# alexkreimer/libviso

Hardware: AMD Instinct MI355X
Metric: stereo_frames_per_sec_1241x376_matcher (higher is better)
Workload: dtype u16; 1 GPU; configs[1]: synthetic 1241x376 stereo pairs, 2000 features/image, SAD matcher only (pack + 3 match_desc/frame + sort)

## Files before the change

### libviso_amd/csrc/common.h

```cpp
#pragma once
#include <hip/hip_runtime.h>
#include <stdint.h>
#include <stddef.h>
#include <atomic>

#include "../../include/viso_hip.h"

#define VISO_ROW 128
#define VISO_ROW8 128
#define VISO_ROW8_SLACK(S) (((1 << (S)) - 1) * VISO_ROW8)
#define VISO_R8_C128 0
#define VISO_R8_ROWS 3
#define VISO_R8_DEFAULT 3
#define VISO_R8_EVERY 16
#define VISO_PACK_SUMS 1
#define VISO_PACK_ROWS8 2
#define VISO_BIAS 32768
#define VISO_WAVE 64
#define VISO_QCAP 256
#define VISO_QPB 32
#define VISO_MATCH_THREADS 256
#define VISO_KPCAP 768
#define VISO_NB 256
#define VISO_SORT_MAX 16384

void viso_set_error(const char* fmt, ...);

#define HIP_TRY(expr)                                                              \
    do {                                                                           \
        hipError_t _e = (expr);                                                    \
        if (_e != hipSuccess) {                                                    \
            viso_set_error("%s:%d: %s -> %s", __FILE__, __LINE__, #expr,           \
                           hipGetErrorString(_e));                                 \
            return VISO_ERR_HIP;                                                   \
        }                                                                          \
    } while (0)

#define VISO_TRY(expr)                                                             \
    do {                                                                           \
        const int _r = (expr);                                                     \
        if (_r < 0) return _r;                                                     \
    } while (0)

struct MatchParamsDev {
    int epi, second, K, _pad;
    float radius, _padf;
    double F[9];
    double sampson_thresh, ratio;
};

struct ImageView {
    const float2* kp;
    const float* frows;
    const int* n;
    float2* skp;
    int* sidx;
    int* rank;
    int* bstart;
    float* xinfo;
    uint8_t* qord;
    uint16_t* rows;
    uint2* sums;
    uint8_t* rows8;
    int* bad;
};

struct MatchProblem {
    ImageView q, t;
    int2* res;
    int* sorted;
    int* pos;
    int* m_cnt;
    unsigned long long* scored;
    int2* ovf;
    int* ovf_cnt;
    int* tile_flag;
    int pidx;
    int cap;
};

struct SolverParamsDev {
    double base, f, cu, cv, inlier_threshold, thresh;
    int ransac_iter, _pad;
};

enum ScratchSlot {
    SLOT_GEN0 = 0, SLOT_GEN1, SLOT_GEN2,
    SLOT_HARRIS_TMP_RESP,
    SLOT_HYP_WORDS,
    SLOT_HYP_TR,
    SLOT_GEN6,
    SLOT_HARRIS_STRIPS,
    SLOT_RANSAC_QUEUE,
    SLOT_RANSAC_ROT,
    SLOT_UNUSED10, SLOT_UNUSED11, SLOT_UNUSED12, SLOT_UNUSED13,
    SLOT_PLAIN_IN, SLOT_PLAIN_OUT,
    SLOT_CIRCLE_TAB,
    SLOT_SUBPIX_IMG, SLOT_SUBPIX_KP, SLOT_SUBPIX_LIST, SLOT_SUBPIX_UV,
// ... 351 lines not shown
```

### libviso_amd/csrc/match.hip

```cpp
#include "common.h"
#include <stdlib.h>
#include "match_dev.h"

#include <math.h>

#ifndef VISO_IMG_THREADS
#define VISO_IMG_THREADS 512
#endif
#ifndef VISO_KP_REGS
#define VISO_KP_REGS 4
#endif

#ifdef VISO_DEBUG_VARIANTS
__device__ unsigned long long viso_dbg_sortkp_clk[8];
extern "C" int viso_debug_sortkp_clocks(unsigned long long* out8) {
    (void)hipDeviceSynchronize();
    return hipMemcpyFromSymbol(out8, HIP_SYMBOL(viso_dbg_sortkp_clk), sizeof(unsigned long long) * 8, 0, hipMemcpyDeviceToHost) == hipSuccess ? VISO_OK : VISO_ERR_HIP;
}
#define SK_CLK(I) do { if (blockIdx.x == 0 && threadIdx.x == 0) viso_dbg_sortkp_clk[I] = wall_clock64(); } while (0)
#else
#define SK_CLK(I) do {} while (0)
#endif
struct KpImport2 { KpImport k[2]; };
__global__ __launch_bounds__(VISO_IMG_THREADS) void sort_kp_kernel(const ImageView* imgs, int n_img, int n64_alloc,
// ... 747 lines not shown
            const int blo = bucket_of<VISO_NB>(xa - r - slack, x0, scale);
            const int bhi = bucket_of<VISO_NB>(xb + r + slack, x0, scale);
            win.lo = P.t.bstart[blo];
            win.W = P.t.bstart[bhi + 1] - win.lo;
        }
    }
    win.cap = min(win.W, VISO_KPCAP);
    for (int w = threadIdx.x; w < win.cap; w += VISO_MATCH_THREADS) {
        s_kp[w] = P.t.skp[win.lo + w];
        s_idx[w] = P.t.sidx[win.lo + w];
    }
    float2 kp0 = make_float2(0.f, 0.f);
    const bool has0 = n2 > 0;
    if (has0) kp0 = P.t.skp[P.t.rank[0]];
    __syncthreads();
    unsigned long long scored = 0;
    for (int j = q0 + wave; j < q1; j += VISO_MATCH_WAVES) {
        QueryResult r;
        const bool done = match_query<GENERAL, false, EPI>(P, mp, j, win, kp0, has0, s_queue[wave], lane, a.dlen, scored, r);
        if (lane == 0) {
            if (done) {
                bool accept = r.idx >= 0;
                if (accept && mp.second) accept = r.bd1 < r.bd2 * mp.ratio;
                P.res[P.q.sidx[j]] = make_int2(accept ? r.idx : -1, r.dist);
            } else {
                P.ovf[atomicAdd(P.ovf_cnt, 1)] = make_int2(prob, j);
            }
        }
    }
    if (lane == 0 && scored) atomicAdd(P.scored, scored);
}

template <bool GENERAL, int EPI>
__global__ __attribute__((amdgpu_waves_per_eu(GENERAL ? 4 : 8, 8))) __launch_bounds__(VISO_MATCH_THREADS) void match_kernel(MatchArgs a) {
    __shared__ __attribute__((aligned(16))) uint2 s_queue[VISO_MATCH_WAVES][VISO_QCAP];
    __shared__ float2 s_kp[VISO_KPCAP];
    __shared__ int s_idx[VISO_KPCAP];
    __shared__ float s_xr[2];
    if constexpr (GENERAL) {
        if (*a.bad == 0) return;
        for (int vb = blockIdx.x; vb < a.vblocks; vb += gridDim.x) {
            __syncthreads();
            match_tile_slot<GENERAL, EPI>(a, vb, s_queue, s_kp, s_idx, s_xr);
        }
    } else {
        match_tile_slot<GENERAL, EPI>(a, blockIdx.x, s_queue, s_kp, s_idx, s_xr);
    }
}

#define VISO_OVF_GRID 4096
#define VISO_OVF_STAGE 768

template <bool GENERAL>
__global__ __launch_bounds__(VISO_WAVE) void match_overflow_kernel(MatchArgs a) {
    __shared__ __attribute__((aligned(16))) uint2 s_queue[VISO_QCAP];
    __shared__ __attribute__((aligned(16))) uint4 s_stage[VISO_OVF_STAGE];
    if (GENERAL && *a.bad == 0) return;
    const int n_ovf = *a.ovf_cnt;
    const int lane = threadIdx.x;
    for (int k = (int)blockIdx.x; k < n_ovf; k += (int)gridDim.x) {
        const int2 e = a.ovf_q[k];
        const MatchProblem P = a.probs[e.x];
        if (((*P.q.bad | *P.t.bad) != 0) != GENERAL) continue;
        const int j = e.y;
        const int n2 = *P.t.n;
        const MatchParamsDev& mp = a.mp[P.pidx];
        float2 kp0 = make_float2(0.f, 0.f);
        const bool has0 = n2 > 0;
        if (has0) kp0 = P.t.skp[P.t.rank[0]];
        unsigned long long scored = 0;
        Window win;
        win.gkp = P.t.skp; win.gidx = P.t.sidx; win.skp = nullptr; win.sidx = nullptr;
        win.lo = 0; win.W = 0; win.cap = 0;
        {
            const float qx = P.q.skp[j].x, r = mp.radius;
            if (n2 > 0 && r >= 0.f) {
                if (qx == qx) {
                    const float slack = (2.f * fabsf(qx) + fabsf(r)) * 1e-6f + 1e-6f;
                    const float x0 = P.t.xinfo[0], scale = P.t.xinfo[1];
                    win.lo = P.t.bstart[bucket_of<VISO_NB>(qx - r - slack, x0, scale)];
                    win.W = P.t.bstart[bucket_of<VISO_NB>(qx + r + slack, x0, scale) + 1] - win.lo;
                }
            }
        }
        QueryResult r;
        match_query<GENERAL, true, -1>(P, mp, j, win, kp0, has0, s_queue, lane, a.dlen, scored, r, s_stage, VISO_OVF_STAGE);
        if (lane == 0) {
            bool accept = r.idx >= 0;
            if (accept && mp.second) accept = r.bd1 < r.bd2 * mp.ratio;
            P.res[P.q.sidx[j]] = make_int2(accept ? r.idx : -1, r.dist);
            if (scored) atomicAdd(P.scored, scored);
        }
        __builtin_amdgcn_wave_barrier();
    }
}

const char* matcher_kernel_name(int variant) {
    return variant == 2 ? "match_batch_kernel<0>" : variant == 3 ? "match_union_kernel" : variant == 5 ? "match_prune_kernel" : variant == 6 ? "match_union8_kernel" : "match_strip_kernel";
}

int launch_match(hipStream_t s, const MatchProblem* probs_dev, int n_probs, int cap_max,
                 int dlen, const MatchParamsDev mp[2], int* bad,
                 hipEvent_t e0, hipEvent_t e1, int layout, int variant,
                 const int2* ovf_q, const int* ovf_cnt, int r8s, int general_possible, int kinds) {
    if (n_probs <= 0 || cap_max <= 0) return VISO_OK;
    variant = matcher_effective(variant, dlen);
    MatchArgs a;
    a.probs = probs_dev;
    a.n_probs = n_probs;
    a.bpp = (cap_max + VISO_QPB - 1) / VISO_QPB;
    a.dlen = dlen;
    a.gs = 1; a.gf = 0; a.gc = 1;
    a.bad = bad;
    a.ovf_q = ovf_q; a.ovf_cnt = ovf_cnt;
    a.mp[0] = mp[0];
    a.mp[1] = mp[1];
    const int groups = (n_probs + 7) / 8;
    const long long blocks = (long long)groups * 8 * a.bpp;
    if (blocks > 0x7fffffffLL) { viso_set_error("matcher grid too large"); return VISO_ERR_UNSUPPORTED; }
    a.vblocks = (int)blocks;
    if (e0) HIP_TRY(hipEventRecord(e0, s));
    {
        const int r = launch_match_batch(s, probs_dev, n_probs, cap_max, mp, bad, layout, e1, variant, r8s, kinds);
        if (r < 0) return r;
    }
    const unsigned gblocks = (unsigned)(blocks < 512 ? blocks : 512);
    if (general_possible && (kinds & VISO_KIND_ALL) == VISO_KIND_ALL) {
        hipLaunchKernelGGL((match_kernel<true, -1>), dim3(gblocks), dim3(VISO_MATCH_THREADS), 0, s, a);
        HIP_TRY(hipGetLastError());
    } else if (general_possible && (kinds & VISO_KIND_TEMPORAL)) {
        hipLaunchKernelGGL((match_kernel<true, 0>), dim3(gblocks), dim3(VISO_MATCH_THREADS), 0, s, a);
        HIP_TRY(hipGetLastError());
    } else if (general_possible && (kinds & VISO_KIND_STEREO)) {
        hipLaunchKernelGGL((match_kernel<true, 1>), dim3(gblocks), dim3(VISO_MATCH_THREADS), 0, s, a);
        HIP_TRY(hipGetLastError());
    }
    hipLaunchKernelGGL(match_overflow_kernel<false>, dim3(VISO_OVF_GRID), dim3(VISO_WAVE), 0, s, a);
    HIP_TRY(hipGetLastError());
    if (general_possible) {
        hipLaunchKernelGGL(match_overflow_kernel<true>, dim3(VISO_OVF_GRID), dim3(VISO_WAVE), 0, s, a);
        HIP_TRY(hipGetLastError());
    }
    return VISO_OK;
}


#define VISO_SORT_THREADS 512
#define VISO_SORT_NB 2048
#define VISO_SORT_FINE 1024
#define VISO_SORT_BMAX 128
#define VISO_SORT_FAST_MAX 8192

__device__ __forceinline__ void sort_tri_row(const TriItem& T, const SolverParamsDev& sp, int r, int i1, int i2) {
    const float2 a = T.kp1[i1], b = T.kp2[i2];
    const double uL = a.x, vL = a.y, uR = b.x, vR = b.y;
    T.x[0 * T.ld + r] = uL; T.x[1 * T.ld + r] = vL; T.x[2 * T.ld + r] = uR; T.x[3 * T.ld + r] = vR;
    if (T.X) {
        const double d = uL - uR;
        T.X[0 * T.ld + r] = sp.base * (uL - sp.cu) / d;
        T.X[1 * T.ld + r] = sp.base * (vL - sp.cv) / d;
        T.X[2 * T.ld + r] = sp.f * sp.base / d;
    }
}

#ifdef VISO_DEBUG_VARIANTS
__device__ unsigned long long viso_dbg_sortm_clk[12];
extern "C" int viso_debug_sortm_clocks(unsigned long long* out12) {
    (void)hipDeviceSynchronize();
    return hipMemcpyFromSymbol(out12, HIP_SYMBOL(viso_dbg_sortm_clk), sizeof(unsigned long long) * 12, 0, hipMemcpyDeviceToHost) == hipSuccess ? VISO_OK : VISO_ERR_HIP;
}
#define SM_CLK(I) do { if (blockIdx.x == 1 && threadIdx.x == 0) viso_dbg_sortm_clk[I] = wall_clock64(); } while (0)
#else
#define SM_CLK(I) do {} while (0)
#endif
__global__ __launch_bounds__(VISO_SORT_THREADS) void sort_matches_kernel(const MatchProblem* probs,
                                                                         int n_probs, int npad_alloc, int fast, int flagged_empty,
                                                                         const TriItem* tri, SolverParamsDev tri_sp) {
    extern __shared__ __attribute__((aligned(16))) unsigned char smem[];
    unsigned long long* keys = reinterpret_cast<unsigned long long*>(smem);
    __shared__ int s_cnt;
    __shared__ int s_start[VISO_SORT_NB + 1];
    __shared__ uint32_t s_red[2][VISO_SORT_THREADS / 64];
    __shared__ unsigned long long s_sum[VISO_SORT_THREADS / 64];
    __shared__ int s_maxb;
    const int prob = blockIdx.x;
    if (prob >= n_probs) return;
    SM_CLK(0);
    const MatchProblem P = probs[prob];
    const bool do_tri = tri != nullptr && prob == 0;
    TriItem T{};
    if (do_tri) T = *tri;
    if (flagged_empty && (*P.q.bad | *P.t.bad) != 0) { if (threadIdx.x == 0) *P.m_cnt = 0; return; }
    const int n1 = *P.q.n;
    const int lane = threadIdx.x & 63, wv = threadIdx.x >> 6;
    if (threadIdx.x == 0) s_cnt = 0;
// ... 109 lines not shown
                const int2 rr = P.res[i1];
                P.sorted[3 * r + 0] = i1;
                P.sorted[3 * r + 1] = rr.x;
                P.sorted[3 * r + 2] = (int)(uint32_t)(k >> 32);
                P.pos[i1] = r;
                if (do_tri) sort_tri_row(T, tri_sp, r, i1, rr.x);
            }
            SM_CLK(7);
            return;
        }
#undef SORT_BUCKET
    }
    int npad = 64;
    while (npad < mv) npad <<= 1;
    for (int i = mv + threadIdx.x; i < npad; i += VISO_SORT_THREADS) keys[i] = ~0ull;
    __syncthreads();
    bitonic_sort_lds<VISO_SORT_THREADS>(keys, npad);
    for (int r = threadIdx.x; r < mv; r += VISO_SORT_THREADS) {
        const unsigned long long k = keys[r];
        const int i1 = (int)(uint32_t)k;
        const int2 rr = P.res[i1];
        P.sorted[3 * r + 0] = i1;
        P.sorted[3 * r + 1] = rr.x;
        P.sorted[3 * r + 2] = (int)(uint32_t)(k >> 32);
        P.pos[i1] = r;
        if (do_tri) sort_tri_row(T, tri_sp, r, i1, rr.x);
    }
}

int launch_sort(hipStream_t s, const MatchProblem* probs_dev, int n_probs, int cap_max, int flagged_empty, const TriItem* tri, const SolverParamsDev* tri_sp) {
    if (n_probs <= 0) return VISO_OK;
    if (cap_max > VISO_SORT_MAX) {
        viso_set_error("match_desc: more than %d queries per call is not supported by this build", VISO_SORT_MAX);
        return VISO_ERR_UNSUPPORTED;
    }
    int npad = 64;
    while (npad < cap_max) npad <<= 1;
    const int fast = npad <= VISO_SORT_FAST_MAX ? 1 : 0;
    const size_t lds = (size_t)npad * sizeof(unsigned long long) * (fast ? 2 : 1) + 16;
    if (lds > 40 * 1024)
        HIP_TRY(hipFuncSetAttribute((const void*)sort_matches_kernel, hipFuncAttributeMaxDynamicSharedMemorySize, (int)lds));
    SolverParamsDev sp{};
    if (tri && tri_sp) sp = *tri_sp;
    hipLaunchKernelGGL(sort_matches_kernel, dim3(n_probs), dim3(VISO_SORT_THREADS), lds, s, probs_dev, n_probs, npad, fast, flagged_empty,
                       tri_sp ? tri : nullptr, sp);
    HIP_TRY(hipGetLastError());
    return VISO_OK;
}

void fill_match_params(MatchParamsDev* d, const viso_match_params* h) {
    d->epi = h->enforce_epipolar != 0;
    d->second = h->enforce_2nd_best != 0;
    d->K = h->max_neighbors;
    d->_pad = 0;
    d->radius = (float)h->radius;
    if (d->radius == 0.f) d->radius = 0.f;
    d->_padf = 0;
    for (int i = 0; i < 9; ++i) d->F[i] = h->F[i];
    d->sampson_thresh = h->sampson_thresh;
    d->ratio = h->ratio_2nd_best;
}
```

### libviso_amd/csrc/match_batch.hip

```cpp
#include "common.h"
#include <stdlib.h>
#include "match_dev.h"

#define MB_THREADS 256
#define MB_WAVES 4
#define MB_QPB 64
#define MB_G 4
#define MB_SEG 128
#define MB_PAD 32
#define MB_KPCAP 512


template <int EPI>
__global__ __attribute__((amdgpu_waves_per_eu(5, 8))) __launch_bounds__(MB_THREADS) void match_batch_kernel(BatchMatchArgs a) {
    __shared__ __attribute__((aligned(16))) uint32_t s_pairs[MB_WAVES][MB_G * MB_SEG + MB_PAD];
    __shared__ __attribute__((aligned(16))) uint32_t s_sads[MB_WAVES][MB_G * MB_SEG + MB_PAD];
    __shared__ __attribute__((aligned(16))) uint32_t s_qrow[MB_WAVES][MB_G][64];
    __shared__ float2 s_kp[MB_KPCAP];
    __shared__ int s_idx[MB_KPCAP];
    __shared__ float s_xr[4];
    if (EPI && a.bad[1] == 0) return;
    for (int vb = blockIdx.x; vb < a.vblocks; vb += gridDim.x) {
    if (vb != (int)blockIdx.x) __syncthreads();
    int prob, qblk;
// ... 236 lines not shown
                sb_ = __builtin_amdgcn_sad_u16(r0[SB].z, b0_.z, sb_);                                      \
                sa_ = __builtin_amdgcn_sad_u16(r0[SA].w, a0_.w, sa_);                                      \
                sb_ = __builtin_amdgcn_sad_u16(r0[SB].w, b0_.w, sb_);                                      \
                sa_ = __builtin_amdgcn_sad_u16(r1[SA].x, a1_.x, sa_);                                      \
                sb_ = __builtin_amdgcn_sad_u16(r1[SB].x, b1_.x, sb_);                                      \
                sa_ = __builtin_amdgcn_sad_u16(r1[SA].y, a1_.y, sa_);                                      \
                sb_ = __builtin_amdgcn_sad_u16(r1[SB].y, b1_.y, sb_);                                      \
                sa_ = __builtin_amdgcn_sad_u16(r1[SA].z, a1_.z, sa_);                                      \
                sb_ = __builtin_amdgcn_sad_u16(r1[SB].z, b1_.z, sb_);                                      \
                sa_ = __builtin_amdgcn_sad_u16(r1[SA].w, a1_.w, sa_);                                      \
                sb_ = __builtin_amdgcn_sad_u16(r1[SB].w, b1_.w, sb_);                                      \
                sa_ += wave_dpp<0xB1>(sa_);                                                                \
                sb_ += wave_dpp<0xB1>(sb_);                                                                \
                sa_ += wave_dpp<0x4E>(sa_);                                                                \
                sb_ += wave_dpp<0x4E>(sb_);                                                                \
                sa_ += wave_dpp<0x141>(sa_);                                                               \
                sb_ += wave_dpp<0x141>(sb_);                                                               \
                if (sub == 0) { sads[dst[SA]] = sa_; sads[dst[SB]] = sb_; }    \
            } while (0)
            int t = 0;
            for (; t + MB_NP < npass; t += MB_NP) {
#pragma unroll
                for (int p = 0; p < MB_NP; p += 2) {
                    MB_REDUCE2(p, p + 1);
                    MB_ISSUE(p, t + p + MB_NP);
                    MB_ISSUE(p + 1, t + p + 1 + MB_NP);
                }
            }
            if (npass > 0) {
#pragma unroll
                for (int p = 0; p < MB_NP; p += 2) MB_REDUCE2(p, p + 1);
            }
#undef MB_REDUCE2
#undef MB_ISSUE
        }
        __builtin_amdgcn_wave_barrier();
        const int nmax = max(max(seg_n[0], seg_n[1]), max(seg_n[2], seg_n[3]));
        if (EPI && nmax <= 16) {
            const int row = lane >> 4, i16 = lane & 15;
            const int n = row == 0 ? seg_n[0] : row == 1 ? seg_n[1] : row == 2 ? seg_n[2] : seg_n[3];
            const int st = row == 0 ? 0 : row == 1 ? c1 : row == 2 ? c2 : c3;
            const int my_orig = row == 0 ? orig[0] : row == 1 ? orig[1] : row == 2 ? orig[2] : orig[3];
            const bool valid = i16 < n;
            const uint32_t sv = valid ? sads[st + i16] : 0xffffffffu;
            const uint32_t m1 = row_min_u32(sv);
            const bool eq = valid && sv == m1;
            const unsigned long long em = __ballot(eq);
            const uint32_t emr = (uint32_t)(em >> (16 * row)) & 0xffffu;
            const int c = __popc(emr);
            const uint32_t m2 = row_min_u32(eq ? 0xffffffffu : sv);
            const uint32_t r_d2 = c > 1 ? m1 : m2;
            if (i16 == 0 && my_orig >= 0) {
                const int j = jg + row * MB_WAVES;
                if (((flags >> row) & 1) || (m1 != 0xffffffffu && c > 1)) {
                    P.ovf[atomicAdd(P.ovf_cnt, 1)] = make_int2(prob, j);
                } else {
                    bool accept = m1 != 0xffffffffu;
                    int idx = -1;
                    if (accept) {
                        const uint32_t r_w = (pairs[st + (__ffs((int)emr) - 1)] & 0x3fffffffu) >> 8;
                        if ((int)r_w < wcap) idx = s_idx[r_w]; else idx = P.t.sidx[lo + (int)r_w];
                        if (mp.second) {
                            const double bd2 = r_d2 == 0xffffffffu ? 1.7976931348623157e308 : (double)r_d2;
                            accept = (double)m1 < bd2 * mp.ratio;
                        }
                    }
                    P.res[my_orig] = make_int2(accept ? idx : -1, (int)m1);
                    scored += (unsigned long long)n;
                }
            }
        } else {
    #pragma unroll
            for (int k = 0; k < MB_G; ++k) {
                if (orig[k] < 0) continue;
                const int j = jg + k * MB_WAVES;
                if (flags & (1 << k)) {
                    if (lane == 0) P.ovf[atomicAdd(P.ovf_cnt, 1)] = make_int2(prob, j);
                    continue;
                }
                const int n = seg_n[k], st = k == 0 ? 0 : k == 1 ? c1 : k == 2 ? c2 : c3;
                uint32_t r_d1 = 0xffffffffu, r_d2 = 0xffffffffu, r_w = 0, r_tie = 0;
                for (int b = 0; b < n; b += VISO_WAVE) {
                    const bool valid = (b + lane) < n;
                    const uint32_t s = valid ? sads[st + b + lane] : 0xffffffffu;
                    const uint32_t m1 = wave_min_u32(s);
                    const bool eq = valid && s == m1;
                    const unsigned long long em = __ballot(eq);
                    const int c = __popcll(em);
                    const uint32_t m2 = wave_min_u32(eq ? 0xffffffffu : s);
                    const uint32_t wfirst = (pairs[st + b + (__ffsll((long long)em) - 1)] & 0x3fffffffu) >> 8;
                    const uint32_t o2 = c > 1 ? m1 : m2;
                    if (m1 < r_d1) { r_d2 = min(r_d1, o2); r_d1 = m1; r_w = wfirst; r_tie = c > 1; }
                    else if (m1 == r_d1) { r_d2 = r_d1; r_tie = 1; }
                    else r_d2 = min(r_d2, m1);
                }
                if (lane == 0) {
                    if (r_tie) {
                        P.ovf[atomicAdd(P.ovf_cnt, 1)] = make_int2(prob, j);
                    } else {
                        bool accept = r_d1 != 0xffffffffu;
                        int idx = -1;
                        if (accept) {
                            if ((int)r_w < wcap) idx = s_idx[r_w]; else idx = P.t.sidx[lo + (int)r_w];
                            if (mp.second) {
                                const double bd2 = r_d2 == 0xffffffffu ? 1.7976931348623157e308 : (double)r_d2;
                                accept = (double)r_d1 < bd2 * mp.ratio;
                            }
                        }
                        P.res[orig[k]] = make_int2(accept ? idx : -1, (int)r_d1);
                        scored += (unsigned long long)n;
                    }
                }
            }

        }
    }
    scored += (unsigned long long)__shfl_xor((long long)scored, 16);
    scored += (unsigned long long)__shfl_xor((long long)scored, 32);
    if (lane == 0 && scored) atomicAdd(P.scored, scored);
    }
}

int launch_match_batch(hipStream_t s, const MatchProblem* probs_dev, int n_probs, int cap_max,
                       const MatchParamsDev mp[2], int* bad, int layout, hipEvent_t e_mid, int variant, int r8s, int kinds) {
    BatchMatchArgs a;
    a.probs = probs_dev;
    a.n_probs = n_probs;
    a.bpp = (cap_max + MB_QPB - 1) / MB_QPB;
    a.gs = 1; a.gf = 0; a.gc = 1; a.vblocks = 0;
    a.bad = bad;
    a.r8s = r8s; a._pad8 = 0;
    a.mp[0] = mp[0];
    a.mp[1] = mp[1];
    const int groups = (n_probs + 7) / 8;
    long long bt = (long long)groups * 8 * a.bpp, bs = bt;
    BatchMatchArgs at = a, as = a;
    if (layout == 1) {
        const int g3 = (groups + 2) / 3;
        at.gs = 3; at.gf = 1; at.gc = 2; bt = (long long)g3 * 2 * 8 * a.bpp;
        as.gs = 3; as.gf = 0; as.gc = 1; bs = (long long)g3 * 8 * a.bpp;
    }
    if (bt > 0x7fffffffLL || bs > 0x7fffffffLL) { viso_set_error("matcher grid too large"); return VISO_ERR_UNSUPPORTED; }
    if (variant == 6 && (kinds & VISO_KIND_ALL) == VISO_KIND_ALL && bt <= VISO_FRAME_MAX_BLOCKS && !e_mid) {
        static const int off = [] { const char* e = getenv("VISO_FRAME_KERNEL"); return e && *e == '0'; }();
        if (!off) {
            const int r = launch_match_frame(s, at, as, bt, cap_max);
            if (r < 0) return r;
            if (kinds & VISO_KIND_NO_WIDE) return VISO_OK;
            as.vblocks = (int)bs;
            hipLaunchKernelGGL((match_batch_kernel<1>), dim3((unsigned)(bs < 1024 ? bs : 1024)), dim3(MB_THREADS), 0, s, as);
// ... 53 lines not shown
```

### libviso_amd/csrc/match_prune.hip

```cpp
#include "common.h"
#include "match_dev.h"

#define MP_THREADS 256
#define MP_WAVES 4
#define MP_QPB 64
#define MP_G 8
#ifndef MP_QSTRIDE
#define MP_QSTRIDE 64
#endif
#ifndef MP_WPE
#define MP_WPE 4
#endif
#ifndef MP_NP
#define MP_NP 2
#endif
#define MP_UCAP 448
#define MP_CCAP 480
#define MP_CPAD (8 * MP_NP + 16)
#define MP_LCAP 576
#define MP_KPCAP 512
#define MP_NBY 64

struct MpTrack { uint32_t m1, m2; };
__device__ __forceinline__ void mp_update(MpTrack& t, uint32_t key) {
// ... 353 lines not shown
        __builtin_amdgcn_wave_barrier();
        MpTrack tr;
        tr.m1 = 0xffffffffu; tr.m2 = 0xffffffffu;
        {
            const int npass = (ccnt + 7) >> 3;
            u32x4 r0[MP_NP], r1[MP_NP];
            uint32_t ent[MP_NP];
#define MP_ISSUE(SLOT, T)                                                                                  \
            do {                                                                                           \
                ent[SLOT] = cells[(T) * 8 + g8];                                                           \
                const grow_t row_ = (grow_t)(wrows + ((ent[SLOT] & 0x00ffffffu) | (uint32_t)(sub << 4)));  \
                r0[SLOT] = row_[0];                                                                        \
                r1[SLOT] = row_[8];                                                                        \
            } while (0)
#define MP_REDUCE(SLOT, T)                                                                                 \
            do {                                                                                           \
                const uint32_t k_ = ent[SLOT] >> 29;                                                       \
                const uint32_t s_sad = MP_SADROW(k_, r0[SLOT], r1[SLOT]);                                  \
                const int c_ = (T) * 8 + g8;                                                               \
                const bool mine_ = k_ == (uint32_t)sub && c_ < ccnt;                                       \
                mp_update(tr, mine_ ? ((s_sad << 9) | (uint32_t)c_) : 0xffffffffu);                        \
            } while (0)
            if (npass > 0) {
#pragma unroll
                for (int p = 0; p < MP_NP; ++p) MP_ISSUE(p, p);
            }
            int t = 0;
            for (; t + MP_NP < npass; t += MP_NP) {
#pragma unroll
                for (int p = 0; p < MP_NP; ++p) {
                    MP_REDUCE(p, t + p);
                    __builtin_amdgcn_sched_barrier(0);
                    MP_ISSUE(p, t + p + MP_NP);
                    __builtin_amdgcn_sched_barrier(0);
                }
            }
            if (npass > 0) {
#pragma unroll
                for (int p = 0; p < MP_NP; ++p) MP_REDUCE(p, t + p);
            }
#undef MP_REDUCE
#undef MP_ISSUE
        }
#pragma unroll
        for (int m = 8; m < VISO_WAVE; m <<= 1) {
            MpTrack o;
            o.m1 = (uint32_t)__shfl_xor((int)tr.m1, m);
            o.m2 = (uint32_t)__shfl_xor((int)tr.m2, m);
            mp_merge(tr, o);
        }
        if (lane < MP_G && my_orig >= 0) {
            const bool none = tr.m1 == 0xffffffffu;
            const uint32_t d1 = tr.m1 >> 9;
            const bool tie = !none && tr.m2 != 0xffffffffu && (tr.m2 >> 9) == d1;
            if (list_ovf || my_cnt > K || tie) {
                P.ovf[atomicAdd(P.ovf_cnt, 1)] = make_int2(prob, my_j);
            } else {
                bool accept = !none;
                int idx = -1;
                if (accept) {
                    const int w = (int)((cells[tr.m1 & 511u] >> 8) & 0xffffu);
                    idx = P.t.sidx[lo + w];
                    if (mp.second) {
                        const double bd2 = tr.m2 == 0xffffffffu ? 1.7976931348623157e308 : (double)(tr.m2 >> 9);
                        accept = (double)d1 < bd2 * mp.ratio;
                    }
                }
                P.res[my_orig] = make_int2(accept ? idx : -1, none ? -1 : (int)d1);
                scored += (unsigned long long)my_cnt;
            }
        }
        __builtin_amdgcn_wave_barrier();
    }
#undef MP_SADROW
#pragma unroll
    for (int m = 1; m < MP_G; m <<= 1) scored += (unsigned long long)__shfl_xor((long long)scored, m);
    if (lane == 0 && scored) atomicAdd(P.scored, scored);
}

int launch_match_prune_temporal(hipStream_t s, const BatchMatchArgs& a, long long blocks) {
    hipLaunchKernelGGL(match_prune_kernel, dim3((unsigned)blocks), dim3(MP_THREADS), 0, s, a);
    hipError_t e = hipGetLastError();
    if (e != hipSuccess) { viso_set_error("match_prune_kernel launch: %s", hipGetErrorString(e)); return VISO_ERR_HIP; }
    return VISO_OK;
}
```

### libviso_amd/csrc/match_stereo.hip

```cpp
#include "common.h"
#include "match_dev.h"

#define ST_THREADS 256
#define ST_WAVES 4
#define ST_QPW 64
#define ST_WCAP 384
#define ST_NBY 64
#define ST_SLOTS 8
#define ST_PCAP (ST_QPW * ST_SLOTS)
#ifndef ST_NP
#define ST_NP 2
#endif
#define ST_PAD (8 * ST_NP)
#define ST_BAND_MAX 6.0f

struct StWaveLds {
    float2 ykp[ST_WCAP];
    uint16_t ypos[ST_WCAP];
    int hist[ST_NBY + 1];
    uint16_t slot[ST_SLOTS][ST_QPW];
    uint32_t flat[ST_PCAP + ST_PAD];
};
static_assert(ST_WCAP <= 512, "window positions share a word with the SAD");

// ... 196 lines not shown
                    __builtin_amdgcn_sched_barrier(0);
                    ST_ISSUE(p, t + p + ST_NP);
                    __builtin_amdgcn_sched_barrier(0);
                }
            }
            if (npass > 0) {
#pragma unroll
                for (int p = 0; p < ST_NP; ++p) ST_REDUCE(p);
            }
#undef ST_REDUCE
#undef ST_ISSUE
        }
        __builtin_amdgcn_wave_barrier();
        ST_CLK(5);
        for (int s = 0; s < n2g; ++s) {
            const uint32_t f = L.flat[base + s];
            const uint32_t v = f >> 9;
            const uint32_t w = (f & 0x1ffu) + (uint32_t)cb;
            const bool lt = v < d1, eq = v == d1;
            d2 = (v <= d1) ? d1 : min(d2, v);
            bw = lt ? w : bw;
            tie = lt ? 0u : (eq ? 1u : tie);
            d1 = min(d1, v);
        }
        nscored += n2g;
        __builtin_amdgcn_wave_barrier();
        if (!__any(seen > skip + ST_SLOTS)) break;
        }
    }
    ST_CLK(6);
    int cnt = cnt_ub;
    {
        unsigned long long need = __ballot(live && cnt_ub > K);
        while (need) {
            const int ql = __ffsll((long long)need) - 1;
            need &= need - 1;
            const float qx = readlane_f32(qv.x, ql);
            const float qy = readlane_f32(qv.y, ql);
            const uint32_t th = (uint32_t)__builtin_amdgcn_readlane((int)thr, ql);
            int c = 0;
            for (int base = 0; base < W; base += VISO_WAVE) {
                const int w = base + lane;
                bool in = false;
                if (w < W) in = __float_as_uint(l1_kp(qx, qy, P.t.skp[lo + w])) < th;
                c += __popcll(__ballot(in));
            }
            if (lane == ql) cnt = c;
        }
    }
    ST_CLK(7);
    unsigned long long scored = 0;
    if (live) {
        const bool none = d1 == 0xffffffffu;
        if (cnt > K || (!none && tie)) {
            P.ovf[atomicAdd(P.ovf_cnt, 1)] = make_int2(prob, j);
        } else {
            bool accept = !none;
            int idx = -1;
            if (accept) {
                idx = P.t.sidx[lo + (int)bw];
                if (mp.second) {
                    const double bd2 = d2 == 0xffffffffu ? 1.7976931348623157e308 : (double)d2;
                    accept = (double)d1 < bd2 * mp.ratio;
                }
            }
            P.res[orig] = make_int2(accept ? idx : -1, (int)d1);
            scored = (unsigned long long)nscored;
        }
    }
    scored = viso_wave_sum63(scored);
    if (lane == 63 && scored) atomicAdd(P.scored, scored);
}

#ifndef ST_NO_LAUNCHER
int launch_match_stereo(hipStream_t s, const BatchMatchArgs& a64, int cap_max) {
    BatchMatchArgs a = a64;
    const int tiles = (cap_max + ST_QPW - 1) / ST_QPW;
    a.bpp = (tiles + ST_WAVES - 1) / ST_WAVES;
    const int groups = (a.n_probs + 7) / 8;
    long long blocks = (long long)groups * 8 * a.bpp;
    if (a.gs == 3) blocks = (long long)((groups + 2) / 3) * a.gc * 8 * a.bpp;
    if (blocks > 0x7fffffffLL) { viso_set_error("matcher grid too large"); return VISO_ERR_UNSUPPORTED; }
    hipLaunchKernelGGL(match_stereo_kernel, dim3((unsigned)blocks), dim3(ST_THREADS), 0, s, a);
    hipError_t e = hipGetLastError();
    if (e != hipSuccess) { viso_set_error("match_stereo_kernel launch: %s", hipGetErrorString(e)); return VISO_ERR_HIP; }
    return VISO_OK;
}
#endif
```

### libviso_amd/csrc/match_union.hip

```cpp
#include "common.h"
#include "match_dev.h"

#define MU_THREADS 256
#define MU_WAVES 4
#define MU_QPB 64
#define MU_G 8
#define MU_UCAP 448
#define MU_PAD 32
#ifndef MU_NP
#define MU_NP 2
#endif
#define MU_KPCAP 512
#define MU_NBY 64

struct MuTrack { uint32_t m1, m2; };

__device__ __forceinline__ void mu_update(MuTrack& t, uint32_t key) {
    t.m2 = med3_u32(t.m1, t.m2, key);
    t.m1 = min(t.m1, key);
}

__device__ __forceinline__ void mu_merge(MuTrack& a, const MuTrack& b) {
    const uint32_t hi = max(a.m1, b.m1);
    a.m2 = min(hi, min(a.m2, b.m2));
// ... 264 lines not shown
                MU_X4x4(s0_, s1_, s2_, s3_, s4_, s5_, s6_, s7_);    \
                const uint32_t c0_ = MU_X2(s0_, s2_), c1_ = MU_X2(s4_, s6_);                               \
                const uint32_t m_ = MU_X1(c0_, c1_);                                                       \
                mu_update(tr, (m_ << 9) | un[SLOT]);                                                       \
            } while (0)
            if (npass > 0) {
#pragma unroll
                for (int p = 0; p < MU_NP; ++p) MU_ISSUE(p, p);
            }
            int t = 0;
            for (; t + MU_NP < npass; t += MU_NP) {
#pragma unroll
                for (int p = 0; p < MU_NP; ++p) {
                    MU_REDUCE(p);
                    __builtin_amdgcn_sched_barrier(0);
                    MU_ISSUE(p, t + p + MU_NP);
                    __builtin_amdgcn_sched_barrier(0);
                }
            }
            if (npass > 0) {
                MU_REDUCE(0);
                if (MU_NP > 1 && t + 1 < npass) MU_REDUCE(MU_NP > 1 ? 1 : 0);
            }
#undef MU_REDUCE
#undef MU_X4x4
#undef MU_X2
#undef MU_X1
#undef MU_SAD
#undef MU_ISSUE
        }
        {
            MuTrack o;
            o.m1 = wave_dpp<0x128>(tr.m1);
            o.m2 = wave_dpp<0x128>(tr.m2);
            mu_merge(tr, o);
            o.m1 = wave_swizzle<0x401F>(tr.m1);
            o.m2 = wave_swizzle<0x401F>(tr.m2);
            mu_merge(tr, o);
            const auto h1 = __builtin_amdgcn_permlane32_swap(tr.m1, tr.m1, false, false);
            const auto h2 = __builtin_amdgcn_permlane32_swap(tr.m2, tr.m2, false, false);
            tr.m1 = h1[0]; tr.m2 = h2[0];
            o.m1 = h1[1]; o.m2 = h2[1];
            mu_merge(tr, o);
        }
        {
            const int k = qslot;
            const int src = ((k & 1) << 2) | (k & 2) | (k >> 2);
            tr.m1 = (uint32_t)__shfl((int)tr.m1, src);
            tr.m2 = (uint32_t)__shfl((int)tr.m2, src);
        }
        const bool mine = (lane & 28) == 0 && my_orig >= 0;
        const bool none = tr.m1 == 0xffffffffu;
        const uint32_t d1 = tr.m1 >> 9;
        const bool tie = !none && tr.m2 != 0xffffffffu && (tr.m2 >> 9) == d1;
        const bool slow = nu > K || __any(mine && tie);
        int my_cnt = 0;
        if (slow) {
            for (int b = 0; b < nu; b += VISO_WAVE) {
                const uint32_t e = (b + lane) < nu ? ul[b + lane] : 0xffffffffu;
#pragma unroll
                for (int k = 0; k < MU_G; ++k) {
                    const int c = __popcll(__ballot(((e >> (31 - k)) & 1u) == 0));
                    if (lane == qlane(k)) my_cnt += c;
                }
            }
        } else if (!list_ovf) {
            scored += ntest - ncnt;
        }
        if (mine) {
            if (list_ovf || my_cnt > K || tie) {
                P.ovf[atomicAdd(P.ovf_cnt, 1)] = make_int2(prob, my_j);
            } else {
                bool accept = !none;
                int idx = -1;
                if (accept) {
                    const int w = (int)((ul[tr.m1 & 511u] >> 8) & 0xffffu);
                    idx = P.t.sidx[lo + w];
                    if (mp.second) {
                        const double bd2 = tr.m2 == 0xffffffffu ? 1.7976931348623157e308 : (double)(tr.m2 >> 9);
                        accept = (double)d1 < bd2 * mp.ratio;
                    }
                }
                P.res[my_orig] = make_int2(accept ? idx : -1, none ? -1 : (int)d1);
                if (slow) scored += (unsigned long long)my_cnt;
            }
        }
    }
#pragma unroll
    for (int m = 1; m < VISO_WAVE; m <<= 1) scored += (unsigned long long)__shfl_xor((long long)scored, m);
    if (lane == 0 && scored) atomicAdd(P.scored, scored);
}

int launch_match_union_temporal(hipStream_t s, const BatchMatchArgs& a, long long blocks) {
    hipLaunchKernelGGL(match_union_kernel, dim3((unsigned)blocks), dim3(MU_THREADS), 0, s, a);
    hipError_t e = hipGetLastError();
    if (e != hipSuccess) { viso_set_error("match_union_kernel launch: %s", hipGetErrorString(e)); return VISO_ERR_HIP; }
    return VISO_OK;
}
```

### libviso_amd/csrc/match_union8.hip

```cpp
#include "common.h"
#include "match_dev.h"
#include <stddef.h>
#include <stdlib.h>

#define MU_THREADS 256
#define MU_WAVES 4
#define MU_QPB 64
#define MU_G 8
#define MU_UCAP 448
#define MU_PAD 32
#ifndef MU_NP
#define MU_NP 2
#endif
#ifndef MU_RNP
#define MU_RNP 2
#endif
#define MU_S8ROWS 176
#define MU_KPCAP 512
#define MU_NBY 64

struct MuTrack { uint32_t m1, m2, m3; };

__device__ __forceinline__ void mu_update(MuTrack& t, uint32_t key) {
    t.m3 = med3_u32(t.m2, t.m3, key);
// ... 342 lines not shown
            const auto h3 = __builtin_amdgcn_permlane32_swap(tr.m3, tr.m3, false, false);
            tr.m1 = h1[0]; tr.m2 = h2[0]; tr.m3 = h3[0];
            o.m1 = h1[1]; o.m2 = h2[1]; o.m3 = h3[1];
            mu_merge(tr, o);
        }
        {
            const int k = lane >> 3;
            const int src = (lane & 0x38) | (k & 1) | ((k & 2) << 1) | ((k & 4) >> 1);
            tr.m1 = (uint32_t)__shfl((int)tr.m1, src);
            tr.m2 = (uint32_t)__shfl((int)tr.m2, src);
            tr.m3 = (uint32_t)__shfl((int)tr.m3, src);
        }
        const bool none = tr.m1 == 0xffffffffu;
        const bool has2 = tr.m2 != 0xffffffffu, has3 = tr.m3 != 0xffffffffu;
        uint32_t dA = 0, dB = 0;
        const uint32_t eA = ul[none ? 0u : (tr.m1 & 511u)], eB = ul[has2 ? (tr.m2 & 511u) : 0u];
        if (__any(!none)) {
            const grow_t ra = (grow_t)(wrows + (((eA & 0x00ffffffu) << 1) | (uint32_t)(sub << 4)));
            const grow_t rb = (grow_t)(wrows + (((eB & 0x00ffffffu) << 1) | (uint32_t)(sub << 4)));
            const grow_t rq = (grow_t)(qrows + ((uint32_t)min(gq_j, q1 - 1) * (uint32_t)(VISO_ROW * 2) + (uint32_t)(sub << 4)));
            const u32x4 a0 = ra[0], a1 = ra[8], b0 = rb[0], b1 = rb[8], x0 = rq[0], x1 = rq[8];
#define MU_SAD16(R0, R1)                                                                                   \
            ({                                                                                             \
                uint32_t s_ = __builtin_amdgcn_sad_u16((R0).x, x0.x, 0u);                                  \
                s_ = __builtin_amdgcn_sad_u16((R0).y, x0.y, s_);                                           \
                s_ = __builtin_amdgcn_sad_u16((R0).z, x0.z, s_);                                           \
                s_ = __builtin_amdgcn_sad_u16((R0).w, x0.w, s_);                                           \
                s_ = __builtin_amdgcn_sad_u16((R1).x, x1.x, s_);                                           \
                s_ = __builtin_amdgcn_sad_u16((R1).y, x1.y, s_);                                           \
                s_ = __builtin_amdgcn_sad_u16((R1).z, x1.z, s_);                                           \
                s_ = __builtin_amdgcn_sad_u16((R1).w, x1.w, s_);                                           \
                s_ += wave_dpp<0xB1>(s_);                                                    \
                s_ += wave_dpp<0x4E>(s_);                                                    \
                s_ += wave_swizzle<0x101F>(s_);                                              \
                s_;                                                                                        \
            })
            dA = MU_SAD16(a0, a1);
            dB = MU_SAD16(b0, b1);
#undef MU_SAD16
        }
        const bool mine = sub == 0 && gq_orig >= 0;
        uint32_t kA = none ? 0xffffffffu : ((dA << 9) | (tr.m1 & 511u)), kB = has2 ? ((dB << 9) | (tr.m2 & 511u)) : 0xffffffffu;
        bool accept = !none, irregular = false, rescue = false;
        if (!none && has2) {
            const uint32_t d1 = min(dA, dB), d2 = max(dA, dB);
            const int L3 = (int)((tr.m3 >> 9) << r8s) - VISO_ROW8_SLACK(r8s);
            if (mp.second) {
                const double lim = (double)d2 * mp.ratio;
                accept = (double)d1 < lim;
                if (has3) rescue = !(accept ? (L3 > (int)d1 && (double)d1 < (double)L3 * mp.ratio) : ((double)L3 >= lim));
            } else if (has3) {
                rescue = !(L3 > (int)d1);
            }
            if (dA == dB) { irregular = true; rescue = false; }
        } else if (!none && mp.second) {
            accept = (double)dA < 1.7976931348623157e308 * mp.ratio;
        }
        {
            asm volatile("" ::: "memory");
            unsigned long long rm = __ballot(rescue && sub == 0);
            const int g8 = lane >> 3;
            uint16_t* ml = reinterpret_cast<uint16_t*>(&s_qrow[wave][0][0]);
            uint32_t* qst = &s_qrow[wave][4][0];
            static_assert(MU_S8ROWS <= 256, "the survivor list holds every position that may survive");
            if (nu > MU_S8ROWS) {
                rm = 0;
                if (rescue) { irregular = true; rescue = false; }
            }
#define MU_UPD2(KEY) do { const uint32_t k_ = (KEY); m2 = med3_u32(m1, m2, k_); m1 = min(m1, k_); } while (0)
            while (rm) {
                const int bit = __builtin_ctzll(rm);
                rm &= rm - 1;
                const int k = bit >> 3;
                const int jq = min(__builtin_amdgcn_readlane(gq_j, bit), q1 - 1);
                const uint32_t ka = (uint32_t)__builtin_amdgcn_readlane((int)kA, bit), kb = (uint32_t)__builtin_amdgcn_readlane((int)kB, bit);
                const uint32_t pa = ka & 511u, pb = kb & 511u;
                const int d1k = (int)(min(ka, kb) >> 9);
                const double limk = (double)(max(ka, kb) >> 9) * mp.ratio;
                const bool acck = !mp.second || (double)d1k < limk;
                const uint32_t msk = 31u - (uint32_t)k;
                const int r8q = mu_r8s();
                const uint32_t qv = *(const __attribute__((address_space(1))) uint32_t*)(qrows + ((uint32_t)jq * (uint32_t)(VISO_ROW * 2) + (uint32_t)(lane << 2)));
                __builtin_amdgcn_wave_barrier();
                int nm = 0;
                for (int b = 0; b < nu; b += VISO_WAVE) {
                    const uint32_t i = (uint32_t)(b + lane);
                    bool sel = false;
                    if (i < (uint32_t)nu) {
                        const uint32_t e = ul[i];
                        const uint32_t q8 = s_s8[wave][k][i];
                        const int Lt = (int)(q8 << (7 + r8q)) - VISO_ROW8_SLACK(r8q);
                        const bool clear = q8 == 255u || (!mp.second ? Lt > d1k : (acck ? (Lt > d1k && (double)d1k < (double)Lt * mp.ratio) : ((double)Lt >= limk)));
                        sel = ((e >> msk) & 1u) == 0 && !clear && i != pa && i != pb;
                        if (sel) s_s8[wave][k][i] = 255;
                    }
                    const unsigned long long bal = __ballot(sel);
                    if (sel) ml[nm + mbcnt(bal)] = (uint16_t)i;
                    nm += __popcll(bal);
                }
                __builtin_amdgcn_wave_barrier();
                qst[lane] = qv;
                if (nm > 0 && lane < 8 * MU_RNP) ml[nm + lane] = ml[nm - 1];
                __builtin_amdgcn_wave_barrier();
                uint32_t m1 = 0xffffffffu, m2 = 0xffffffffu;
                if (nm > 0) {
                    for (int t = 0; t * 8 < nm; t += MU_RNP) {
                        uint32_t pos[MU_RNP];
                        u32x4 a0[MU_RNP], a1[MU_RNP];
#pragma unroll
                        for (int p = 0; p < MU_RNP; ++p) {
                            pos[p] = ml[(t + p) * 8 + g8];
                            const grow_t ra = (grow_t)(wrows + (((ul[pos[p]] & 0x00ffffffu) << 1) | (uint32_t)(sub << 4)));
                            a0[p] = ra[0]; a1[p] = ra[8];
                        }
#pragma unroll
                        for (int p = 0; p < MU_RNP; ++p) {
                            int o_ = sub * 4;
                            asm volatile("" : "+v"(o_));
                            const u32x4 x0_ = *reinterpret_cast<const u32x4*>(&qst[o_]);
                            uint32_t sa = __builtin_amdgcn_sad_u16(a0[p].x, x0_.x, 0u);
                            sa = __builtin_amdgcn_sad_u16(a0[p].y, x0_.y, sa);
                            sa = __builtin_amdgcn_sad_u16(a0[p].z, x0_.z, sa);
                            sa = __builtin_amdgcn_sad_u16(a0[p].w, x0_.w, sa);
                            const u32x4 x1_ = *reinterpret_cast<const u32x4*>(&qst[o_ + 32]);
                            sa = __builtin_amdgcn_sad_u16(a1[p].x, x1_.x, sa);
                            sa = __builtin_amdgcn_sad_u16(a1[p].y, x1_.y, sa);
                            sa = __builtin_amdgcn_sad_u16(a1[p].z, x1_.z, sa);
                            sa = __builtin_amdgcn_sad_u16(a1[p].w, x1_.w, sa);
                            sa += wave_dpp<0xB1>(sa);
                            sa += wave_dpp<0x4E>(sa);
                            sa += wave_swizzle<0x101F>(sa);
                            MU_UPD2(((t + p) * 8 + g8 < nm && sub == 0) ? ((sa << 9) | pos[p]) : 0xffffffffu);
                        }
                    }
#define MU_MRG2(O1, O2) do { const uint32_t o1_ = (O1), o2_ = (O2); m2 = min(max(m1, o1_), min(m2, o2_)); m1 = min(m1, o1_); } while (0)
                    MU_MRG2(wave_dpp<0x128>(m1), wave_dpp<0x128>(m2));
                    MU_MRG2(wave_swizzle<0x401F>(m1), wave_swizzle<0x401F>(m2));
                    {
                        const auto h1 = __builtin_amdgcn_permlane32_swap(m1, m1, false, false);
                        const auto h2 = __builtin_amdgcn_permlane32_swap(m2, m2, false, false);
                        m1 = h1[0]; m2 = h2[0];
                        MU_MRG2(h1[1], h2[1]);
                    }
#undef MU_MRG2
                }
                bool again = false;
                if (g8 == k) {
                    MU_UPD2(kA);
                    MU_UPD2(kB);
                    kA = m1; kB = m2;
                    accept = !mp.second || (double)(m1 >> 9) < (double)(m2 >> 9) * mp.ratio;
                    again = accept && !acck;
                }
                if (__any(again)) rm |= 1ull << bit;
            }
#undef MU_UPD2
            if (rescue && (kA >> 9) == (kB >> 9)) irregular = true;
        }
        const uint32_t kwin = min(kA, kB);
        const uint32_t d1 = kwin >> 9;
        const uint32_t ewin = ul[none ? 0u : (kwin & 511u)];
        const bool slow = nu > K || __any(mine && irregular);
        int my_cnt = 0;
        if (slow) {
            for (int b = 0; b < nu; b += VISO_WAVE) {
                const uint32_t e = (b + lane) < nu ? ul[b + lane] : 0xffffffffu;
#pragma unroll
                for (int k = 0; k < MU_G; ++k) {
                    const int c = __popcll(__ballot(((e >> (31 - k)) & 1u) == 0));
                    if ((lane >> 3) == k) my_cnt += c;
                }
            }
        } else if (!list_ovf) {
            scored += ntest - ncnt;
        }
        if (mine) {
            if (list_ovf || my_cnt > K || irregular) {
                P.ovf[atomicAdd(P.ovf_cnt, 1)] = make_int2(prob, gq_j);
            } else {
                int idx = -1;
                if (accept) {
                    const int w = (int)((ewin & 0x00ffffffu) >> 7);
                    idx = P.t.sidx[lo + w];
                }
                P.res[gq_orig] = make_int2(idx, none ? -1 : (int)d1);
                if (slow) scored += (unsigned long long)my_cnt;
            }
        }
        MU_CLK(2 + r);
    }
    scored = viso_wave_sum63(scored);
    if (lane == 63 && scored) atomicAdd(P.scored, scored);
}

#ifndef MU_NO_LAUNCHER
int launch_match_union8_temporal(hipStream_t s, const BatchMatchArgs& a, long long blocks) {
    size_t pad = 0;
#ifdef VISO_DEBUG_VARIANTS
    { static const int p = [] { const char* e = getenv("VISO_EXP_U8_LDS_PAD"); return e ? atoi(e) : 0; }(); if (p > 0 && p < 32768) pad = (size_t)p; }
#endif
    hipLaunchKernelGGL(match_union8_kernel, dim3((unsigned)blocks), dim3(MU_THREADS), pad, s, a);
    hipError_t e = hipGetLastError();
    if (e != hipSuccess) { viso_set_error("match_union8_kernel launch: %s", hipGetErrorString(e)); return VISO_ERR_HIP; }
    return VISO_OK;
}
#endif
```

Before: 537,000 frames/s.

## Skip overflow rescans for distance ties when ratio test rejects ties anyway

Adds a tie_rejects flag, set when the second-best ratio test is enabled with ratio <= 1. With that flag set, queries whose best and second-best distances tie are resolved directly in every fast matcher variant instead of being pushed to the overflow queue, because such a tie is rejected regardless of which index wins. The overflow path is also merged into a single kernel launch that branches per entry on the general/bad flag, replacing two launches. This cuts overflow traffic and one launch, but depends on the tie always ending in rejection so results stay the same.

```diff
diff --git a/libviso_amd/csrc/common.h b/libviso_amd/csrc/common.h
--- a/libviso_amd/csrc/common.h
+++ b/libviso_amd/csrc/common.h
@@ -43,7 +43,8 @@
     } while (0)
 
 struct MatchParamsDev {
-    int epi, second, K, _pad;
+    int epi, second, K;
+    int tie_rejects;
     float radius, _padf;
     double F[9];
     double sampson_thresh, ratio;
diff --git a/libviso_amd/csrc/match.hip b/libviso_amd/csrc/match.hip
--- a/libviso_amd/csrc/match.hip
+++ b/libviso_amd/csrc/match.hip
@@ -823,45 +823,49 @@
 #define VISO_OVF_STAGE 768
 
 template <bool GENERAL>
+__device__ __forceinline__ void match_overflow_entry(const MatchArgs& a, const MatchProblem& P, int j, int lane, uint2* s_queue, uint4* s_stage) {
+    const int n2 = *P.t.n;
+    const MatchParamsDev& mp = a.mp[P.pidx];
+    float2 kp0 = make_float2(0.f, 0.f);
+    const bool has0 = n2 > 0;
+    if (has0) kp0 = P.t.skp[P.t.rank[0]];
+    unsigned long long scored = 0;
+    Window win;
+    win.gkp = P.t.skp; win.gidx = P.t.sidx; win.skp = nullptr; win.sidx = nullptr;
+    win.lo = 0; win.W = 0; win.cap = 0;
+    {
+        const float qx = P.q.skp[j].x, r = mp.radius;
+        if (n2 > 0 && r >= 0.f) {
+            if (qx == qx) {
+                const float slack = (2.f * fabsf(qx) + fabsf(r)) * 1e-6f + 1e-6f;
+                const float x0 = P.t.xinfo[0], scale = P.t.xinfo[1];
+                win.lo = P.t.bstart[bucket_of<VISO_NB>(qx - r - slack, x0, scale)];
+                win.W = P.t.bstart[bucket_of<VISO_NB>(qx + r + slack, x0, scale) + 1] - win.lo;
+            }
+        }
+    }
+    QueryResult r;
+    match_query<GENERAL, true, -1>(P, mp, j, win, kp0, has0, s_queue, lane, a.dlen, scored, r, s_stage, VISO_OVF_STAGE);
+    if (lane == 0) {
+        bool accept = r.idx >= 0;
+        if (accept && mp.second) accept = r.bd1 < r.bd2 * mp.ratio;
+        P.res[P.q.sidx[j]] = make_int2(accept ? r.idx : -1, r.dist);
+        if (scored) atomicAdd(P.scored, scored);
+    }
+}
+
+template <bool WITH_GENERAL>
 __global__ __launch_bounds__(VISO_WAVE) void match_overflow_kernel(MatchArgs a) {
     __shared__ __attribute__((aligned(16))) uint2 s_queue[VISO_QCAP];
     __shared__ __attribute__((aligned(16))) uint4 s_stage[VISO_OVF_STAGE];
-    if (GENERAL && *a.bad == 0) return;
     const int n_ovf = *a.ovf_cnt;
     const int lane = threadIdx.x;
     for (int k = (int)blockIdx.x; k < n_ovf; k += (int)gridDim.x) {
         const int2 e = a.ovf_q[k];
         const MatchProblem P = a.probs[e.x];
-        if (((*P.q.bad | *P.t.bad) != 0) != GENERAL) continue;
-        const int j = e.y;
-        const int n2 = *P.t.n;
-        const MatchParamsDev& mp = a.mp[P.pidx];
-        float2 kp0 = make_float2(0.f, 0.f);
-        const bool has0 = n2 > 0;
-        if (has0) kp0 = P.t.skp[P.t.rank[0]];
-        unsigned long long scored = 0;
-        Window win;
-        win.gkp = P.t.skp; win.gidx = P.t.sidx; win.skp = nullptr; win.sidx = nullptr;
-        win.lo = 0; win.W = 0; win.cap = 0;
-        {
-            const float qx = P.q.skp[j].x, r = mp.radius;
-            if (n2 > 0 && r >= 0.f) {
-                if (qx == qx) {
-                    const float slack = (2.f * fabsf(qx) + fabsf(r)) * 1e-6f + 1e-6f;
-                    const float x0 = P.t.xinfo[0], scale = P.t.xinfo[1];
-                    win.lo = P.t.bstart[bucket_of<VISO_NB>(qx - r - slack, x0, scale)];
-                    win.W = P.t.bstart[bucket_of<VISO_NB>(qx + r + slack, x0, scale) + 1] - win.lo;
-                }
-            }
-        }
-        QueryResult r;
-        match_query<GENERAL, true, -1>(P, mp, j, win, kp0, has0, s_queue, lane, a.dlen, scored, r, s_stage, VISO_OVF_STAGE);
-        if (lane == 0) {
-            bool accept = r.idx >= 0;
-            if (accept && mp.second) accept = r.bd1 < r.bd2 * mp.ratio;
-            P.res[P.q.sidx[j]] = make_int2(accept ? r.idx : -1, r.dist);
-            if (scored) atomicAdd(P.scored, scored);
-        }
+        const bool general = __builtin_amdgcn_readfirstlane((*P.q.bad | *P.t.bad) != 0 ? 1 : 0) != 0;
+        if (!general) match_overflow_entry<false>(a, P, e.y, lane, s_queue, s_stage);
+        else if (WITH_GENERAL) match_overflow_entry<true>(a, P, e.y, lane, s_queue, s_stage);
         __builtin_amdgcn_wave_barrier();
     }
 }
@@ -906,12 +910,9 @@
         hipLaunchKernelGGL((match_kernel<true, 1>), dim3(gblocks), dim3(VISO_MATCH_THREADS), 0, s, a);
         HIP_TRY(hipGetLastError());
     }
-    hipLaunchKernelGGL(match_overflow_kernel<false>, dim3(VISO_OVF_GRID), dim3(VISO_WAVE), 0, s, a);
+    if (general_possible) hipLaunchKernelGGL(match_overflow_kernel<true>, dim3(VISO_OVF_GRID), dim3(VISO_WAVE), 0, s, a);
+    else hipLaunchKernelGGL(match_overflow_kernel<false>, dim3(VISO_OVF_GRID), dim3(VISO_WAVE), 0, s, a);
     HIP_TRY(hipGetLastError());
-    if (general_possible) {
-        hipLaunchKernelGGL(match_overflow_kernel<true>, dim3(VISO_OVF_GRID), dim3(VISO_WAVE), 0, s, a);
-        HIP_TRY(hipGetLastError());
-    }
     return VISO_OK;
 }
 
@@ -1127,7 +1128,7 @@
     d->epi = h->enforce_epipolar != 0;
     d->second = h->enforce_2nd_best != 0;
     d->K = h->max_neighbors;
-    d->_pad = 0;
+    d->tie_rejects = d->second && h->ratio_2nd_best <= 1.0;
     d->radius = (float)h->radius;
     if (d->radius == 0.f) d->radius = 0.f;
     d->_padf = 0;
diff --git a/libviso_amd/csrc/match_batch.hip b/libviso_amd/csrc/match_batch.hip
--- a/libviso_amd/csrc/match_batch.hip
+++ b/libviso_amd/csrc/match_batch.hip
@@ -312,7 +312,7 @@
             const uint32_t r_d2 = c > 1 ? m1 : m2;
             if (i16 == 0 && my_orig >= 0) {
                 const int j = jg + row * MB_WAVES;
-                if (((flags >> row) & 1) || (m1 != 0xffffffffu && c > 1)) {
+                if (((flags >> row) & 1) || (m1 != 0xffffffffu && c > 1 && !mp.tie_rejects)) {
                     P.ovf[atomicAdd(P.ovf_cnt, 1)] = make_int2(prob, j);
                 } else {
                     bool accept = m1 != 0xffffffffu;
@@ -355,7 +355,7 @@
                     else r_d2 = min(r_d2, m1);
                 }
                 if (lane == 0) {
-                    if (r_tie) {
+                    if (r_tie && !mp.tie_rejects) {
                         P.ovf[atomicAdd(P.ovf_cnt, 1)] = make_int2(prob, j);
                     } else {
                         bool accept = r_d1 != 0xffffffffu;
diff --git a/libviso_amd/csrc/match_prune.hip b/libviso_amd/csrc/match_prune.hip
--- a/libviso_amd/csrc/match_prune.hip
+++ b/libviso_amd/csrc/match_prune.hip
@@ -429,7 +429,7 @@
         if (lane < MP_G && my_orig >= 0) {
             const bool none = tr.m1 == 0xffffffffu;
             const uint32_t d1 = tr.m1 >> 9;
-            const bool tie = !none && tr.m2 != 0xffffffffu && (tr.m2 >> 9) == d1;
+            const bool tie = !none && tr.m2 != 0xffffffffu && (tr.m2 >> 9) == d1 && !mp.tie_rejects;
             if (list_ovf || my_cnt > K || tie) {
                 P.ovf[atomicAdd(P.ovf_cnt, 1)] = make_int2(prob, my_j);
             } else {
diff --git a/libviso_amd/csrc/match_stereo.hip b/libviso_amd/csrc/match_stereo.hip
--- a/libviso_amd/csrc/match_stereo.hip
+++ b/libviso_amd/csrc/match_stereo.hip
@@ -272,7 +272,7 @@
     unsigned long long scored = 0;
     if (live) {
         const bool none = d1 == 0xffffffffu;
-        if (cnt > K || (!none && tie)) {
+        if (cnt > K || (!none && tie && !mp.tie_rejects)) {
             P.ovf[atomicAdd(P.ovf_cnt, 1)] = make_int2(prob, j);
         } else {
             bool accept = !none;
diff --git a/libviso_amd/csrc/match_union.hip b/libviso_amd/csrc/match_union.hip
--- a/libviso_amd/csrc/match_union.hip
+++ b/libviso_amd/csrc/match_union.hip
@@ -340,7 +340,7 @@
         const bool mine = (lane & 28) == 0 && my_orig >= 0;
         const bool none = tr.m1 == 0xffffffffu;
         const uint32_t d1 = tr.m1 >> 9;
-        const bool tie = !none && tr.m2 != 0xffffffffu && (tr.m2 >> 9) == d1;
+        const bool tie = !none && tr.m2 != 0xffffffffu && (tr.m2 >> 9) == d1 && !mp.tie_rejects;
         const bool slow = nu > K || __any(mine && tie);
         int my_cnt = 0;
         if (slow) {
diff --git a/libviso_amd/csrc/match_union8.hip b/libviso_amd/csrc/match_union8.hip
--- a/libviso_amd/csrc/match_union8.hip
+++ b/libviso_amd/csrc/match_union8.hip
@@ -418,7 +418,7 @@
             } else if (has3) {
                 rescue = !(L3 > (int)d1);
             }
-            if (dA == dB) { irregular = true; rescue = false; }
+            if (dA == dB && !mp.tie_rejects) { irregular = true; rescue = false; }
         } else if (!none && mp.second) {
             accept = (double)dA < 1.7976931348623157e308 * mp.ratio;
         }
@@ -521,7 +521,7 @@
                 if (__any(again)) rm |= 1ull << bit;
             }
 #undef MU_UPD2
-            if (rescue && (kA >> 9) == (kB >> 9)) irregular = true;
+            if (rescue && (kA >> 9) == (kB >> 9) && !mp.tie_rejects) irregular = true;
         }
         const uint32_t kwin = min(kA, kB);
         const uint32_t d1 = kwin >> 9;
```

Result: no change. 541,500 frames/s, median of 6 (+0.8%).
